# Darkbblue/generic-diffusion-feature

Hardware: AMD Instinct MI355X
Metric: images/sec feature-extract, SDXL 1024^2 single-timestep (higher is better)
Workload: dtype f16; 1 GPU; SDXL UNet 1024x1024 (latent 128x128), batch 16/GPU, t=100, hooks=config_xl_practical (4 ids, 15.73 MB/img), full forward; global_batch=16, parallelism=dp1 (batch sharded, weights broadcast once), residual_stream=fp32 master + fp16 shadow, launched_by=single process, max_inflight_forwards=0

## Files before the change

generic-diffusion-feature_amd/csrc/gemm.hip:

```cpp
#include "gemm_mainloop_ring.h"
#include "gemm_mainloop_8phase.h"
#include "gemm_epilogue.h"
#include <cstdio>
#include <cstdlib>
#include <cstring>
#include <deque>
#include <mutex>
#include <string>

namespace gdf {

template <int MODE, int BM, int BN, int STAGES, bool GEGLU, bool DIT, bool BF = false, bool QKN = false, bool SPLIT = false, bool MX = false,
          bool GNS = false>
__device__ __forceinline__ void gemm_body(const GemmParams& p) {
  using T = GemmTile<MODE, BM, BN, STAGES, GEGLU, DIT, BF, QKN, SPLIT, MX, GNS>;
  extern __shared__ __attribute__((aligned(16))) char smem[];
  T t(p, smem);
  const int tiles_n = (p.N + BN - 1) / BN;
  const int nblk = ((p.M + BM - 1) / BM) * tiles_n;
  constexpr bool PERSIST = (STAGES == 8);
  int vb = blockIdx.x;
#if defined(GDF_STAGGER)
  if (p.stagger > 0 && (int)blockIdx.x < p.stagger_wgs) {
    const unsigned long long t0 = __builtin_amdgcn_s_memrealtime();
    const unsigned long long d = (unsigned long long)(p.stagger & 0xffffff) * (unsigned)((blockIdx.x >> 3) % (unsigned)(p.stagger >> 24));
    while (__builtin_amdgcn_s_memrealtime() - t0 < d) __builtin_amdgcn_s_sleep(16);
  }
#endif
  do {
  GDF_TR(0); GDF_TR_ID();
  t.locate(vb, tiles_n, nblk);
  f32x4 acc[T::FM][T::FN];
#pragma unroll
  for (int i = 0; i < T::FM; ++i)
#pragma unroll
    for (int j = 0; j < T::FN; ++j) acc[i][j] = f32x4{0.f, 0.f, 0.f, 0.f};
  if constexpr (STAGES == 8) gemm_mainloop_8phase_256(t, acc);
  else if constexpr (STAGES == 9) gemm_mainloop_8phase_320(t, acc);
  else gemm_mainloop_ring(t, acc);
#if defined(GDF_ABLATE_EPI) && GDF_ABLATE_EPI == 2
  wait_vmcnt<0>();
#endif
  __syncthreads();
  GDF_TR(3);
#if defined(GDF_ABLATE_EPI) && GDF_ABLATE_EPI == 1
#pragma unroll
  for (int i = 0; i < T::FM; ++i)
#pragma unroll
    for (int j = 0; j < T::FN; ++j) asm volatile("" ::"v"(acc[i][j]));
#else
  gemm_epilogue(t, acc);
#endif
  GDF_TR(4);
  if constexpr (!PERSIST) break;
  vb += gridDim.x;
  if (vb >= nblk) break;
  asm volatile("s_waitcnt lgkmcnt(0)" ::: "memory");
  __builtin_amdgcn_s_barrier();
  } while (true);
}

template <int MODE, int BM, int BN, int STAGES, bool GEGLU>
__global__ __launch_bounds__(BM * 2, 2) void gemm_kernel(const GemmParams p) {
  gemm_body<MODE, BM, BN, STAGES, GEGLU, false>(p);
}
template <int MODE, int BM, int BN, int STAGES>
__global__ __launch_bounds__(BM * 2, 2) void gemm_gn_kernel(const GemmParams p) {
  gemm_body<MODE, BM, BN, STAGES, false, false, false, false, false, false, true>(p);
}
template <int MODE, int BM, int BN, int STAGES, bool GEGLU>
__global__ __launch_bounds__(BM * 2, 2) void gemm_split_kernel(const GemmParams p) {
  gemm_body<MODE, BM, BN, STAGES, GEGLU, false, false, false, true>(p);
}
template <int BM, int BN, int STAGES, bool BF, bool QKN>
__global__ __launch_bounds__(BM * 2, 2) void gemm_dit_kernel(const GemmParams p) {
  gemm_body<A_DENSE, BM, BN, STAGES, false, true, BF, QKN>(p);
}

template <int BM, int BN, int STAGES, bool BF, bool QKN>
__global__ __launch_bounds__(BM * 2, 2) void gemm_dit_split_kernel(const GemmParams p) {
  gemm_body<A_DENSE, BM, BN, STAGES, false, true, BF, QKN, true>(p);
}

template <int BM, int BN, int STAGES>
__global__ __launch_bounds__(BM * 2, 2) void gemm_mx_kernel(const GemmParams p) {
  gemm_body<A_DENSE, BM, BN, STAGES, false, true, true, false, false, true>(p);
}

static int persist_wgs() {
  static const int off = [] { const char* e = getenv("GDF_PERSIST"); return e && atoi(e) == 0; }();
  if (off) return 1 << 30;
  static std::atomic<int> cus[16];
  int dev = 0;
  if (hipGetDevice(&dev) != hipSuccess || dev < 0 || dev >= 16) return 1 << 30;
  int n = cus[dev].load(std::memory_order_relaxed);
  if (n == 0) {
    if (hipDeviceGetAttribute(&n, hipDeviceAttributeMultiprocessorCount, dev) != hipSuccess || n < 8 || (n & 7)) n = 1 << 30;
    cus[dev].store(n, std::memory_order_relaxed);
  }
  return n;
}

template <int MODE, int BM, int BN, int STAGES, bool GEGLU, bool DIT = false, bool BF = false, bool QKN = false, bool SPLIT = false, bool MX = false,
          bool GNS = false>
static hipError_t launch_t(const GemmParams& p, hipStream_t s) {
  const int tiles_m = (p.M + BM - 1) / BM, tiles_n = (p.N + BN - 1) / BN;
  const int smem = (STAGES >= 8 ? 2 : STAGES) * (BM * 128 + BN * 128);
  static std::atomic<uint64_t> attr_mask{0};
  {
    const void* fn;
    if constexpr (MX) fn = (const void*)gemm_mx_kernel<BM, BN, STAGES>;
    else if constexpr (GNS) fn = (const void*)gemm_gn_kernel<MODE, BM, BN, STAGES>;
    else if constexpr (DIT && SPLIT) fn = (const void*)gemm_dit_split_kernel<BM, BN, STAGES, BF, QKN>;
    else if constexpr (DIT) fn = (const void*)gemm_dit_kernel<BM, BN, STAGES, BF, QKN>;
    else if constexpr (SPLIT) fn = (const void*)gemm_split_kernel<MODE, BM, BN, STAGES, GEGLU>;
    else fn = (const void*)gemm_kernel<MODE, BM, BN, STAGES, GEGLU>;
    const hipError_t e = ensure_dyn_smem(attr_mask, fn, smem);
    if (e != hipSuccess) return e;
  }
  GemmParams q = p;
  q.sb_gm = q.sb_gn = 0;
  if (!p.no_superblock) {
    const int conc = (p.cus > 0 ? p.cus / 8 : 32) * ((BM == 256) ? 1 : 2);
    static const int gn_max = [] { const char* e = getenv("GDF_SB_GN_MAX"); return e ? atoi(e) : 4; }();
    for (int gn = gn_max; gn >= 2; gn >>= 1) {
      const int gm = conc / gn;
      if (tiles_n % gn == 0 && tiles_m % gm == 0 && (tiles_m / gm) * (tiles_n / gn) >= 8 && tiles_n > gn) {
        q.sb_gm = gm; q.sb_gn = gn;
        break;
      }
    }
  }
  int gx = tiles_m * tiles_n;
  const int pw = (p.cus > 0 && p.cus < persist_wgs()) ? p.cus : persist_wgs();
  {
    static const float us = [] { const char* e = getenv("GDF_STAGGER_US"); return e ? (float)atof(e) : 0.f; }();
    static const int min_rounds = [] { const char* e = getenv("GDF_STAGGER_MIN_ROUNDS"); return e ? atoi(e) : 2; }();
    q.stagger = 0; q.stagger_wgs = 0;
    static const int groups = [] { const char* e = getenv("GDF_STAGGER_GROUPS"); return e ? atoi(e) : 2; }();
    if (us > 0.f && groups > 1 && BM == 256 && pw < (1 << 30) && gx >= min_rounds * pw) { q.stagger = (int)(us * 100.f) | (groups << 24); q.stagger_wgs = pw; }
  }
  if (STAGES == 8 && gx > pw && !(p.batch > 1)) gx = pw;
  const dim3 grid(gx, (STAGES == 2 && p.splitk > 1) ? p.splitk : p.batch > 1 ? p.batch : 1);
  if constexpr (MX) hipLaunchKernelGGL((gemm_mx_kernel<BM, BN, STAGES>), grid, dim3(BM * 2), smem, s, q);
  else if constexpr (GNS) hipLaunchKernelGGL((gemm_gn_kernel<MODE, BM, BN, STAGES>), grid, dim3(BM * 2), smem, s, q);
  else if constexpr (DIT && SPLIT) hipLaunchKernelGGL((gemm_dit_split_kernel<BM, BN, STAGES, BF, QKN>), grid, dim3(BM * 2), smem, s, q);
  else if constexpr (DIT) hipLaunchKernelGGL((gemm_dit_kernel<BM, BN, STAGES, BF, QKN>), grid, dim3(BM * 2), smem, s, q);
  else if constexpr (SPLIT) hipLaunchKernelGGL((gemm_split_kernel<MODE, BM, BN, STAGES, GEGLU>), grid, dim3(BM * 2), smem, s, q);
  else hipLaunchKernelGGL((gemm_kernel<MODE, BM, BN, STAGES, GEGLU>), grid, dim3(BM * 2), smem, s, q);
  return hipGetLastError();
}

static double round_fill(long tiles, int slots) {
  if (tiles <= 0) return 0.0;
  const long rounds = (tiles + slots - 1) / slots;
  return (double)tiles / (double)(rounds * slots);
}

static int pick_variant_any(const GemmParams& p);
static bool is_split(const GemmParams& p) { return !p.dit && (p.k_w > 0 || p.o16_lo > 0); }
static bool is_dit_split(const GemmParams& p) { return p.dit && (p.k_w > 0 || p.o16_lo > 0); }
static int pick_variant(const GemmParams& p) {
  const int v = pick_variant_any(p);
  if (is_dit_split(p)) return (v == 8256 || v == 1256) ? 8256 : 128;
  if (!is_split(p) || v == 16) return v;
  if (p.geglu) return v == 825 ? 825 : 128;
  if (p.mode == A_CONV_SMALLC) return v == 160 ? 160 : 128;
  return (v == 932 || v == 160) ? v : 128;
}
static int pick_variant_any(const GemmParams& p) {
  const int S1 = p.cus > 0 ? p.cus : 256, S2 = 2 * S1;
  if (p.dit) {
    const long t256 = (long)((p.M + 255) / 256) * ((p.N + 255) / 256);
    if (p.variant == 128 || p.variant == 1256 || p.variant == 2128 || p.variant == 8256) return p.variant;
    if (t256 >= 128 && (long)((p.N + 255) / 256) * 256 <= (long)p.N + p.N / 8) return 8256;
    return (p.N % 128 == 0 && (long)((p.M + 255) / 256) * (p.N / 128) >= 256) ? 2128 : 128;
  }
  if (p.bn == 16) return 16;
  if (p.splitk > 1) {
    static const int force = [] { const char* e = getenv("GDF_SPLITK_TILE"); return e ? atoi(e) : 0; }();
    if (force == 160 && p.N % 160 == 0) return 160;
    if (force == 128 && p.N % 128 == 0) return 128;
    return (p.N % 160 == 0) ? 160 : 128;
  }
  if (p.variant) return p.variant;
  const long tiles256 = (long)((p.M + 255) / 256) * ((p.N + 127) / 128);
  const long tiles320 = (long)((p.M + 255) / 256) * ((p.N + 319) / 320);
  if (p.geglu) {
    const long tm256 = (p.M + 255) / 256, tm128 = (p.M + 127) / 128;
    double best = 0.0; int bv = 128;
    auto cand = [&](int v, double rate, long tiles, int slots) { const double sc = rate * round_fill(tiles, slots); if (sc > best) { best = sc; bv = v; } };
    if (p.N % 256 == 0) cand(825, 1.00, tm256 * (p.N / 256), S1);
    if (p.N % 320 == 0) cand(320, 0.95, tm256 * (p.N / 320), S1);
    cand(256, 0.80, tm256 * ((p.N + 127) / 128), S1);
    cand(128, 0.70, tm128 * ((p.N + 127) / 128), S2);
// ... 4 lines not shown
      const double s932 = 1.00 * round_fill(tiles320, S1), s160 = 0.85 * round_fill((long)((p.M + 127) / 128) * (p.N / 160), S2);
      const double s128 = 0.70 * round_fill((long)((p.M + 127) / 128) * ((p.N + 127) / 128), S2);
      return (s932 >= s160 && s932 >= s128) ? 932 : (s160 >= s128 ? 160 : 128);
    }
    if (p.N % 160 == 0) return 160;
    if (p.N % 256 == 0 && (long)((p.M + 255) / 256) * (p.N / 256) >= 256) return 826;
    return (p.N <= 128 && p.M >= (1 << 20)) ? 256 : 128;
  }
  if (p.res32 && p.K <= 1536 && p.N % 160 == 0 && tiles320 <= S2 &&
      !(p.N % 320 == 0 && p.N >= 640 && p.K >= 640 && tiles320 % S1 == 0)) return 160;
  if (p.N % 320 == 0) {
    const double s932 = 1.00 * round_fill(tiles320, S1), s160 = 0.87 * round_fill((long)((p.M + 127) / 128) * (p.N / 160), S2);
    const double s128 = 0.72 * round_fill((long)((p.M + 127) / 128) * ((p.N + 127) / 128), S2);
    return (s932 >= s160 && s932 >= s128) ? 932 : (s160 >= s128 ? 160 : 128);
  }
  if (p.N % 160 == 0 && p.K >= 1024) return 160;
  if ((long)p.M * p.N >= (1L << 26) && tiles256 >= S2) return 256;
  return 128;
}

bool gemm_qkn_ok(int M, int N, int K) {
  GemmParams g{}; g.M = M; g.N = N; g.K = K; g.dit = 1; g.mode = A_DENSE;
  const int v = pick_variant(g);
  return v == 8256 || v == 1256;
}

const char* gemm_kernel_name(const GemmParams& p) {
  const int v = pick_variant(p);
  int bm = 128, bn = 128, st = 2;
  if (v == 16) bn = 16; else if (v == 160) bn = 160; else if (v == 256) { bm = 256; st = 3; } else if (v == 320) { bm = 256; bn = 320; }
  else if (v == 825) { bm = 256; bn = 256; st = 8; } else if (v == 932) { bm = 256; bn = 320; st = 9; } else if (v == 826) { bm = 256; bn = 256; st = 8; }
  if (p.mode == A_CONV_SMALLC && v != 160) { bm = 128; bn = 128; st = 2; }
  char tmp[64];
  if (p.gn_partial && !p.dit) snprintf(tmp, sizeof tmp, "gemm_gn_kernel<%d, %d, %d, %d>", p.mode, bm, bn, st);
  else if (p.dit && p.mx) snprintf(tmp, sizeof tmp, "gemm_mx_kernel<256, 256, 8>");
  else if (p.dit) snprintf(tmp, sizeof tmp, "%s<%d, %d, %d, %s, %s>", is_dit_split(p) ? "gemm_dit_split_kernel" : "gemm_dit_kernel", v == 128 ? 128 : 256, (v == 1256 || v == 8256) ? 256 : 128, v == 8256 ? 8 : v == 2128 ? 3 : 2, p.bf16 ? "true" : "false", p.qkn_nq ? "true" : "false");
  else snprintf(tmp, sizeof tmp, "%s<%d, %d, %d, %d, %s>", is_split(p) ? "gemm_split_kernel" : "gemm_kernel", p.mode, bm, bn, st, p.geglu ? "true" : "false");
  static std::mutex mu;
  static std::deque<std::string> names;
  std::lock_guard<std::mutex> lk(mu);
  for (const std::string& n : names) if (n == tmp) return n.c_str();
  names.emplace_back(tmp);
  return names.back().c_str();
}

int gemm_gn_slab_rows(const GemmParams& p) {
  if ((p.mode != A_CONV3 && p.mode != A_CONV_SMALLC) || p.dit || p.geglu || p.splitk > 1 || p.batch > 1 || is_split(p) || p.bn == 16) return 0;
  if ((p.M % 64) != 0 || (p.N % 8) != 0) return 0;
  const int v = pick_variant(p);
  if (p.mode == A_CONV_SMALLC) return v != 160 ? 64 : 0;
  if (v == 932) return (p.M % 128) == 0 ? 128 : 0;
  return (v == 128 || v == 160 || v == 256 || v == 826) ? 64 : 0;
}

hipError_t launch_gemm(const GemmParams& p, hipStream_t s) {
  if (p.M <= 0 || p.N <= 0) return hipSuccess;
  if (p.mode != A_CONV_SMALLC && (p.K % BK) != 0) return hipErrorInvalidValue;
  if (p.mode == A_CONV3 && (p.Cin % BK) != 0) return hipErrorInvalidValue;
  if (p.k_w > 0 && (p.K != 2 * p.k_w || (p.k_w % BK) != 0 || p.mode == A_CONV_SMALLC || (p.dit && !p.bf16) || (p.mode == A_CONV3 && (p.k_w % (9 * BK)) != 0)))
    return hipErrorInvalidValue;
  if (p.o16_lo > 0 && ((p.dit && !p.bf16) || p.bn == 16 || (p.o16_lo % 8) != 0)) return hipErrorInvalidValue;
  if (p.out_f16 && !(p.dit && p.bf16)) return hipErrorInvalidValue;
  const int v = pick_variant(p);
  if (v != 16 && ((p.geglu ? p.N / 2 : p.N) % 8) != 0) return hipErrorInvalidValue;
  if (p.bf16 && !p.dit) return hipErrorInvalidValue;
  if (p.gn_partial) {
    if (gemm_gn_slab_rows(p) == 0 || !p.out16) return hipErrorInvalidValue;
    if (p.mode == A_CONV_SMALLC) return launch_t<A_CONV_SMALLC, 128, 128, 2, false, false, false, false, false, false, true>(p, s);
    if (v == 932) return launch_t<A_CONV3, 256, 320, 9, false, false, false, false, false, false, true>(p, s);
    if (v == 160) return launch_t<A_CONV3, 128, 160, 2, false, false, false, false, false, false, true>(p, s);
    if (v == 826) return launch_t<A_CONV3, 256, 256, 8, false, false, false, false, false, false, true>(p, s);
    if (v == 256) return launch_t<A_CONV3, 256, 128, 3, false, false, false, false, false, false, true>(p, s);
    return launch_t<A_CONV3, 128, 128, 2, false, false, false, false, false, false, true>(p, s);
  }
  if (p.dit) {
    if (p.mode != A_DENSE || p.geglu || p.batch > 1) return hipErrorInvalidValue;
    if (p.qkn_nq && ((v != 8256 && v != 1256) || (p.qkn_nq % 128) != 0)) return hipErrorInvalidValue;
    if (p.qkn_nq && (p.res32 || p.res16 || p.rowvec || p.aux16 || p.out32)) return hipErrorInvalidValue;
    if (p.mx) {
      if (!p.bf16 || p.qkn_nq || is_dit_split(p) || (p.N % 8)) return hipErrorInvalidValue;
      return launch_t<A_DENSE, 256, 256, 8, false, true, true, false, false, true>(p, s);
    }
    if (is_dit_split(p)) {
      if (v == 8256) return p.qkn_nq ? launch_t<A_DENSE, 256, 256, 8, false, true, true, true, true>(p, s) : launch_t<A_DENSE, 256, 256, 8, false, true, true, false, true>(p, s);
      return p.qkn_nq ? hipErrorInvalidValue : launch_t<A_DENSE, 128, 128, 2, false, true, true, false, true>(p, s);
    }
    if (p.bf16) {
      if (v == 8256) return p.qkn_nq ? launch_t<A_DENSE, 256, 256, 8, false, true, true, true>(p, s) : launch_t<A_DENSE, 256, 256, 8, false, true, true>(p, s);
      if (v == 1256) return p.qkn_nq ? launch_t<A_DENSE, 256, 256, 2, false, true, true, true>(p, s) : launch_t<A_DENSE, 256, 256, 2, false, true, true>(p, s);
      if (v == 2128) return launch_t<A_DENSE, 256, 128, 3, false, true, true>(p, s);
      return launch_t<A_DENSE, 128, 128, 2, false, true, true>(p, s);
    }
    if (v == 8256) return p.qkn_nq ? launch_t<A_DENSE, 256, 256, 8, false, true, false, true>(p, s) : launch_t<A_DENSE, 256, 256, 8, false, true>(p, s);
    if (v == 1256) return p.qkn_nq ? launch_t<A_DENSE, 256, 256, 2, false, true, false, true>(p, s) : launch_t<A_DENSE, 256, 256, 2, false, true>(p, s);
    if (v == 2128) return launch_t<A_DENSE, 256, 128, 3, false, true>(p, s);
// ... 154 lines not shown
```

generic-diffusion-feature_amd/csrc/gemm_epilogue.h:

```cpp
#pragma once
#include "gemm_tile.h"

namespace gdf {

template <class T>
__device__ __forceinline__ void gemm_epilogue(T& t, f32x4 (&acc)[T::FM][T::FN]) {
  GDF_TILE_GEOMETRY(T);
  GDF_TILE_STATE(t);
  _Float16* const out16 = t.out16;
  const float* const e_res32 = QKN ? nullptr : p.res32;
  const float* const e_rowvec = QKN ? nullptr : p.rowvec;
  const _Float16* const e_res16 = QKN ? nullptr : p.res16;
  _Float16* const e_aux16 = QKN ? nullptr : p.aux16;
  float* const e_out32 = QKN ? nullptr : (STAGES == 2 && p.splitk > 1) ? p.out32 + (size_t)blockIdx.y * p.o32_sstride : p.out32;
  static_assert(!GEGLU || (FN % 2 == 0), "GEGLU needs an even number of column fragments per wave");
  constexpr int FNV = GEGLU ? FN / 2 : FN;
  constexpr int WTNV = FNV * 16;
  constexpr int SLD = WTNV + 4;
  constexpr int PR = (FM * FN >= 32) ? 16 : 32;
  constexpr int PASSES = WTM / PR;
  constexpr int FPP = FM / PASSES;
  float* st = (float*)(smem) + wave * (PR * SLD);
  constexpr int OUTW = WTNV;
  constexpr int LPR = OUTW / 8;
// ... 269 lines not shown
            if (e_aux16) e_aux16[(size_t)row * p.ldaux + col + e] = (_Float16)x;
            if (e_res32) x += e_res32[(size_t)row * p.ldres + col + e];
            else if (e_res16) x += (float)e_res16[(size_t)row * p.ldres + col + e];
            if (out16) out16[(size_t)row * p.ldo16 + col + e] = (_Float16)x;
            if (e_out32) e_out32[(size_t)row * p.ldo32 + col + e] = x;
          }
        }
    }
    __builtin_amdgcn_wave_barrier();
    __builtin_amdgcn_sched_barrier(0);
  }
  if constexpr (GNS) {
    static_assert((WTM == 64 || WTM == 128) && PR * SLD >= 64 * 16, "one slab per wave tile");
#pragma unroll
    for (int e = 0; e < 8; ++e) { st[lane * 16 + e] = gsum[e]; st[lane * 16 + 8 + e] = gsq[e]; }
    __builtin_amdgcn_wave_barrier();
    if (lane < LPR && full && p.gn_partial && m0 + wm * WTM < p.M) {
      float a[16];
#pragma unroll
      for (int e = 0; e < 16; ++e) a[e] = 0.f;
#pragma unroll
      for (int r = 0; r < RPI; ++r)
#pragma unroll
        for (int e = 0; e < 16; ++e) a[e] += st[(r * LPR + lane) * 16 + e];
      const int slab = (m0 + wm * WTM) / WTM;
      f32x4* gp = (f32x4*)(p.gn_partial + ((size_t)slab * p.N + col) * 2);
#pragma unroll
      for (int q = 0; q < 4; ++q) gp[q] = f32x4{a[2 * q], a[8 + 2 * q], a[2 * q + 1], a[8 + 2 * q + 1]};
    }
    __builtin_amdgcn_wave_barrier();
  }
}

}
```

generic-diffusion-feature_amd/csrc/kernels.h:

```cpp
#pragma once
#include <hip/hip_runtime.h>
#include <stdint.h>
#include <atomic>
#include "launch.h"

typedef _Float16 half_t;

namespace gdf {

inline hipError_t ensure_dyn_smem(std::atomic<uint64_t>& mask, const void* fn, int bytes) {
  int dev = 0;
  hipError_t e = hipGetDevice(&dev);
  if (e != hipSuccess) return e;
  const uint64_t bit = 1ull << (dev & 63);
  if (mask.load(std::memory_order_acquire) & bit) return hipSuccess;
  e = hipFuncSetAttribute(fn, hipFuncAttributeMaxDynamicSharedMemorySize, bytes);
  if (e != hipSuccess) return e;
  mask.fetch_or(bit, std::memory_order_release);
  return hipSuccess;
}

#if defined(__HIPCC__)
__device__ __forceinline__ float e16_to_f32(half_t h, int bf) {
  return bf ? __uint_as_float((uint32_t)__builtin_bit_cast(unsigned short, h) << 16) : (float)h;
// ... 38 lines not shown
  int geglu;
  int bn;
  int splitk;
  long o32_sstride;
  int batch;
  long w_bstride;
  long o_bstride;
  int sb_gm, sb_gn;
  int no_superblock;
  int no_early_mma;
  int variant;
  int dit;
  int act;
  int rv_mul;
  int rv_seg_rows, rv_rps2;
  int rv_tok;
  int qkn_nq;
  const float* qkn_wq; const float* qkn_wk; float qkn_eps;
  const float* rope_cos; const float* rope_sin;
  int qkn_pos0, qkn_rps;
  int qkn_seg_rows, qkn_pos1, qkn_rps2;
  int bf16;
  float acc_scale, out16_scale;
  int k_w;
  uint32_t a_lo_bytes;
  int o16_lo;
  int cus;
  int out_f16;
  int mx;
  const float* mx_rowscale;
  const float* mx_colscale;
  float* gn_partial;
  int stagger, stagger_wgs;
};
hipError_t launch_gemm(const GemmParams& p, hipStream_t s);
int gemm_gn_slab_rows(const GemmParams& p);
int gemm_splitk_factor(const GemmParams& p);
hipError_t launch_gemm_splitk(const GemmParams& p, int splitk, float* ws, hipStream_t s);
const char* gemm_kernel_name(const GemmParams& p);
bool gemm_qkn_ok(int M, int N, int K);

struct AttnParams {
  const half_t* q; int ldq;
  const half_t* k; int ldk;
  const half_t* v; int ldv;
  half_t* o; int ldo;
  int B, heads, Sq, Sk, D;
  int kv_bstride;
  float scale;
  half_t* map;
  half_t* map2;
  const int* kv_len;
  int seg_T;
  int bf16;
  int o_lo;
  int o_pair_bf16;
  int q_lo, kv_lo;
  float o_scale;
};
hipError_t launch_attention(const AttnParams& p, hipStream_t s);

size_t gn_partial_floats(int B, int HW, int C);
hipError_t launch_gn_stats(const half_t* x16, const float* x32, int ld, int B, int HW, int C, int G, float eps,
                           const float* gamma, const float* beta, float* partial, float* ab, hipStream_t s, int x_lo = 0);
hipError_t launch_gn_apply(const half_t* x16, const float* x32, int ld, int B, int HW, int C,
                           const float* ab, int silu, half_t* y, hipStream_t s, int x_lo = 0, int ldy = 0, int y_lo = 0);
// ... 59 lines not shown
```

generic-diffusion-feature_amd/csrc/model.cpp:

```cpp
#include "builder.h"
#include <shared_mutex>

namespace gdf {

thread_local std::string g_err;
void set_error(const std::string& s) { g_err = s; }
const char* last_error() { return g_err.c_str(); }

struct ModelBuilder : WeightBuilder {
  explicit ModelBuilder(Model& mm) : WeightBuilder(mm) {}
  ResnetW resnet(const std::string& p, int ci, int co) {
    ResnetW r; r.cin = ci; r.cout = co;
    r.n1 = norm(p + ".norm1", ci);
    r.c1 = conv3(p + ".conv1", co, ci);
    r.temb_off = m.temb_total;
    m.temb_regs.push_back({p + ".time_emb_proj", co, m.temb_total});
    m.temb_total += co;
    r.n2 = norm(p + ".norm2", co);
    r.c2 = conv3(p + ".conv2", co, co);
    r.has_sc = ci != co;
    if (r.has_sc) r.sc = lin(p + ".conv_shortcut", co, ci, true, true);
    return r;
  }

  VitW vit(const std::string& p, int c, int heads, int depth) {
    const GdfArch& a = m.arch;
    VitW v; v.c = c; v.heads = heads;
    v.gn = norm(p + ".norm", c);
    v.pin = lin(p + ".proj_in", c, c, true, !a.use_linear_projection);
    for (int i = 0; i < depth; ++i) {
      const std::string b = p + ".transformer_blocks." + std::to_string(i);
      BlockW w;
      w.ln1 = norm(b + ".norm1", c);
      w.qkv = lin_alloc(3 * c, c, false);
// ... 213 lines not shown
    const size_t gn = groupnorm(x, w.gn, 1e-6f, false, SP_GNV);
    Act tok = new_act(C, x.H, x.W, true);
    {
      Epi e; e.bias = wt(w.pin.b); e.has_bias = true; out_to(e, tok, w.blocks.empty());
      gemm("proj_in", ws(gn), C * p_gnv, n, w.pin, C, C, 0, e, s_gnv * C);
    }
    untmp(gn, img_bytes(n, C, SP_GNV));
    for (size_t bi = 0; bi < w.blocks.size() && !stop; ++bi) {
      const BlockW& bw = w.blocks[bi];
      const std::string bid = id + "-block" + std::to_string(bi);
      const size_t nb = n * C * 2;
      const size_t nb_lna = img_bytes(n, C, SP_LN_ATTN), nb_ao = img_bytes(n, C, SP_ATTN_OUT), nb_ao2 = img_bytes(n, C, SP_ATTN2_OUT), nb_lnf = img_bytes(n, C, SP_LN_FF);
      size_t ln = layernorm(tok, bw.ln1, SP_LN_ATTN);
      const int s_qkv = spl(SP_QKV), lq = 3 * C * (1 + s_qkv);
      const size_t qkv = tmp(n * (size_t)lq * 2);
      { Epi e; e.out16 = ws(qkv); e.has_o16 = true; e.ldo16 = lq; e.o16_lo = s_qkv * 3 * C;
        gemm("attn1_qkv", ws(ln), C * p_lna, n, bw.qkv, 3 * C, C, 0, e, s_lna * C); }
      untmp(ln, nb_lna);
      hook_copy(want(bid + "-self-q", C, x.H, x.W), ws(qkv), lq, n, C);
      hook_copy(want(bid + "-self-k", C, x.H, x.W), ws(qkv + (size_t)C * 2), lq, n, C);
      hook_copy(want(bid + "-self-v", C, x.H, x.W), ws(qkv + (size_t)2 * C * 2), lq, n, C);
      size_t ao = tmp(nb_ao);
      const int ms = maps ? want_map(bid + "-self-map", heads, S, S) : (dry_map(bid + "-self-map"), -1);
      attention("attn1", ws(qkv), lq, ws(qkv + (size_t)C * 2), lq, ws(qkv + (size_t)2 * C * 2), lq, ws(ao), C * p_ao, heads,
                S, S, D, ms, -1, s_ao * C, s_qkv * 3 * C, s_qkv * 3 * C);
      untmp(qkv, n * (size_t)lq * 2);
      { Epi e; e.bias = wt(bw.o1.b); e.has_bias = true; residual_from(e, tok); out_to(e, tok, false);
        gemm("attn1_out", ws(ao), C * p_ao, n, bw.o1, C, C, 0, e, s_ao * C); }
      untmp(ao, nb_ao);
      if (stop) break;
      ln = layernorm(tok, bw.ln2, SP_LN_ATTN);
      const int s_xq = spl(SP_XQKV);
      const int hq = want(bid + "-cross-q", C, x.H, x.W);
      const bool q2_direct = hq >= 0 && !s_xq;
      const size_t q2 = q2_direct ? 0 : tmp(nb * (1 + s_xq));
      const Ref q2r = q2_direct ? Ref{BUF_HOOK0 + hq, 0} : ws(q2);
      { Epi e; e.out16 = q2r; e.has_o16 = true; e.ldo16 = C * (1 + s_xq); e.o16_lo = s_xq * C;
        gemm("attn2_q", ws(ln), C * p_lna, n, bw.q2, C, C, 0, e, s_lna * C); }
      untmp(ln, nb_lna);
      if (q2_direct) hook_done();
      else if (hq >= 0) hook_copy(hq, ws(q2), C * (1 + s_xq), n, C);
      const bool shared = opt.reserved[0] != 0;
      const size_t kv = dry ? 0 : kv_bufs[bw.kv_group].first + (size_t)bw.kv_index * kv_bufs[bw.kv_group].second;
      ao = tmp(nb_ao2);
      const int mc = maps ? want_map(bid + "-cross-map", heads, S, n_ctx) : (dry_map(bid + "-cross-map"), -1);
      attention("attn2", q2r, C * (1 + s_xq), ws(kv), 2 * C * (1 + s_xq), ws(kv + (size_t)C * 2), 2 * C * (1 + s_xq), ws(ao), C * p_ao2, heads, S, n_ctx, D, mc,
                shared ? 0 : n_ctx, s_ao2 * C, s_xq * C, s_xq * 2 * C);
      if (!q2_direct) untmp(q2, nb * (1 + s_xq));
      { Epi e; e.bias = wt(bw.o2.b); e.has_bias = true; residual_from(e, tok); out_to(e, tok, false);
        gemm("attn2_out", ws(ao), C * p_ao2, n, bw.o2, C, C, 0, e, s_ao2 * C); }
      untmp(ao, nb_ao2);
      if (stop) break;
      ln = layernorm(tok, bw.ln3, SP_LN_FF);
      const int hi = want(bid + "-ffn-inner", 4 * C, x.H, x.W);
      const bool direct = hi >= 0 && !s_inn;
      const size_t inner_b = img_bytes(n, 4 * C, SP_FF_INNER);
      const size_t inner = direct ? 0 : tmp(inner_b);
      const Ref innr = direct ? Ref{BUF_HOOK0 + hi, 0} : ws(inner);
      { Epi e; e.bias = wt(bw.ff1.b); e.has_bias = true; e.geglu = geglu_group(8 * C); e.out16 = innr; e.has_o16 = true; e.ldo16 = 4 * C * p_inn;
        e.o16_lo = s_inn * 4 * C;
        gemm("ff_geglu", ws(ln), C * p_lnf, n, bw.ff1, 8 * C, C, 0, e, s_lnf * C); }
      untmp(ln, nb_lnf);
      if (direct) hook_done();
      else if (hi >= 0) hook_copy(hi, innr, 4 * C * p_inn, n, 4 * C);
      {
        const bool shadow = (bi + 1 == w.blocks.size()) || (!dry && P.requested.count(bid + "-out"));
        Epi e; e.bias = wt(bw.ff2.b); e.has_bias = true; residual_from(e, tok); out_to(e, tok, shadow);
        gemm("ff_out", innr, 4 * C * p_inn, n, bw.ff2, C, 4 * C, 0, e, s_inn * 4 * C); }
      if (!direct) untmp(inner, inner_b);
      gather(bid + "-out", tok);
    }
    if (!stop) {
      Epi e; e.bias = wt(w.pout.b); e.has_bias = true; residual_from(e, x); out_to(e, y);
      gemm("proj_out", tok.h, tok.ld, n, w.pout, C, C, 0, e, tok.lo);
    }
    free_act(tok);
    gather(id + "-out", y);
  }
  void dry_map(const std::string& id) { if (dry) P.dry_ids.push_back(id); }

  size_t layernorm(const Act& x, const NormW& w, int out_cls) {
// ... 504 lines not shown
```

generic-diffusion-feature_amd/csrc/ops_api.cpp:

```cpp
#include "../../include/gdf_ops.h"
#include "model.h"

using namespace gdf;

static bool span_ok(size_t a_bytes, size_t w_bytes, const char* what) {
  if (a_bytes < (1ull << 31) && w_bytes < (1ull << 31)) return true;
  set_error(std::string(what) + ": operand larger than 2 GiB (32-bit buffer offsets); split the rows");
  return false;
}

static int fin(hipError_t e, const char* what) {
  if (e == hipSuccess) return GDF_OK;
  set_error(std::string(what) + ": " + hipGetErrorString(e));
  return GDF_ERR_HIP;
}

extern "C" {

int gdf_op_gemm(const void* A, int lda, const void* W, const float* bias, const float* res32, const void* res16,
                int ldres, void* out16, int ldo16, float* out32, int ldo32, int M, int N, int K, int flags,
                void* stream) {
  GemmParams g{};
  if (!span_ok(((size_t)M - 1) * lda * 2 + (size_t)K * 2, (size_t)N * K * 2, "gemm")) return GDF_ERR_UNSUPPORTED;
  g.A = (const half_t*)A; g.lda = lda; g.a_bytes = (uint32_t)(((size_t)M - 1) * lda * 2 + (size_t)K * 2);
// ... 113 lines not shown

int gdf_op_splitk_factor(int M, int N, int K, int conv) {
  GemmParams g{}; g.M = M; g.N = N; g.K = K; g.mode = conv ? A_CONV3 : A_DENSE; g.bn = 128;
  return gemm_splitk_factor(g);
}

int gdf_op_conv_in(const void* x_nchw, int B, int Cin, int H, int W, const void* w_oihw, const float* bias, int Cout,
                   void* out16, void* scratch, void* stream) {
  hipStream_t s = (hipStream_t)stream;
  half_t* lat8 = (half_t*)scratch;
  half_t* w = (half_t*)((char*)scratch + (size_t)B * H * W * 16);
  hipError_t e = launch_pack_latents((const half_t*)x_nchw, B, Cin, H, W, lat8, nullptr, s);
  if (e != hipSuccess) return fin(e, "pack_latents");
  e = launch_relayout_conv(w_oihw, 0, w, Cout, Cin, 9, 8, 16, s);
  if (e != hipSuccess) return fin(e, "relayout");
  GemmParams g{};
  const size_t M = (size_t)B * H * W;
  g.A = lat8; g.lda = 8; g.a_bytes = (uint32_t)(M * 16);
  g.M = (int)M; g.N = Cout; g.K = 128; g.mode = A_CONV_SMALLC; g.H = H; g.W = W; g.OH = H; g.OW = W; g.stride = 1; g.Cin = 8;
  g.Wt = w; g.w_bytes = (uint32_t)((size_t)Cout * 256);
  g.bias = bias; g.out16 = (half_t*)out16; g.ldo16 = Cout; g.bn = 128; g.rows_per_sample = 1;
  return fin(launch_gemm(g, s), "conv_in");
}

int gdf_op_attention(const void* q, int ldq, const void* k, int ldk, const void* v, int ldv, void* o, int ldo,
                     int B, int heads, int Sq, int Sk, int D, void* map, void* stream) {
  AttnParams a{};
  a.q = (const half_t*)q; a.ldq = ldq; a.k = (const half_t*)k; a.ldk = ldk; a.v = (const half_t*)v; a.ldv = ldv;
  a.o = (half_t*)o; a.ldo = ldo; a.B = B; a.heads = heads; a.Sq = Sq; a.Sk = Sk; a.D = D; a.kv_bstride = Sk;
  a.scale = 1.0f / sqrtf((float)D); a.map = (half_t*)map;
  return fin(launch_attention(a, (hipStream_t)stream), "attention");
}

size_t gdf_op_groupnorm_scratch_bytes(int B, int HW, int C) { return gn_partial_floats(B, HW, C) * 4 + (size_t)B * C * 8 + 256; }

int gdf_op_groupnorm(const void* x16, const float* x32, int ld, int B, int HW, int C, int G, float eps,
                     const float* gamma, const float* beta, int silu, void* y, void* scratch, void* stream) {
  hipStream_t s = (hipStream_t)stream;
  if (gn_fused_slab(B, HW, C, G))
    return fin(launch_gn_fused((const half_t*)x16, x32, ld, B, HW, C, G, eps, gamma, beta, silu, (half_t*)y, s), "gn_fused");
  float* partial = (float*)scratch;
  float* ab = partial + (gn_partial_floats(B, HW, C) + 63) / 64 * 64;
  hipError_t e = launch_gn_stats((const half_t*)x16, x32, ld, B, HW, C, G, eps, gamma, beta, partial, ab, s);
  if (e != hipSuccess) return fin(e, "gn_stats");
  return fin(launch_gn_apply((const half_t*)x16, x32, ld, B, HW, C, ab, silu, (half_t*)y, s), "gn_apply");
}

int gdf_op_layernorm(const void* x16, const float* x32, int ld, int R, int C, float eps, const float* gamma,
                     const float* beta, void* y, void* stream) {
  return fin(launch_layernorm((const half_t*)x16, x32, ld, R, C, eps, gamma, beta, (half_t*)y, (hipStream_t)stream), "layernorm");
}

int gdf_op_copy2d(const void* s16, const float* s32, int lds, void* dst, int ldd, int R, int C, void* stream) {
  return fin(launch_copy2d((const half_t*)s16, s32, lds, (half_t*)dst, ldd, R, C, (hipStream_t)stream), "copy2d");
}

int gdf_op_relayout_conv3(const void* w, void* dst, int O, int I, void* stream) {
  return fin(launch_relayout_conv(w, 0, (half_t*)dst, O, I, 9, I, 9, (hipStream_t)stream, 64), "relayout_conv3");
}
int gdf_op_relayout_geglu(const void* w, const float* bias, void* w_dst, float* bias_dst, int R, int K, int group, void* stream) {
  hipError_t e = launch_relayout_rows(w, 0, (half_t*)w_dst, R, K, 0, group, (hipStream_t)stream);
  if (e != hipSuccess) return fin(e, "relayout_geglu");
  if (bias) e = launch_relayout_vec(bias, 1, bias_dst, R, 0, group, (hipStream_t)stream);
  return fin(e, "relayout_geglu_bias");
}

// ... 93 lines not shown
```

include/gdf_ops.h:

```cpp
#ifndef GDF_OPS_H
#define GDF_OPS_H
#include <stddef.h>
#include <stdint.h>
#ifdef __cplusplus
extern "C" {
#endif

int gdf_op_gemm(const void* A, int lda, const void* W, const float* bias, const float* res32, const void* res16,
                int ldres, void* out16, int ldo16, float* out32, int ldo32, int M, int N, int K, int flags,
                void* stream);

int gdf_op_conv3x3(const void* x, int ld, int B, int H, int W, int Cin, const void* Wt, int Cout, const float* bias,
                   const float* rowvec, int stride, int ups, const float* res32, void* aux16, void* out16,
                   float* out32, int narrow , void* stream);

int gdf_op_gemm_split(const void* A, int lda, int a_lo, const void* W, const float* bias, const float* res32, int ldres, void* out16,
                      int ldo16, int o16_lo, float* out32, int ldo32, int M, int N, int Kw, int flags , void* stream);
int gdf_op_conv3x3_split(const void* x, int ld, int a_lo, int B, int H, int W, int Cin, const void* Wt, int Cout, const float* bias,
                         int stride, int ups, const float* res32, void* out16, int ldo16, int o16_lo, float* out32, void* stream);
int gdf_op_layernorm_split(const float* x32, int ld, int R, int C, float eps, const float* gamma, const float* beta, void* y, int ldy,
                           int y_lo, void* stream);
int gdf_op_groupnorm_split(const void* x16, int x_lo, const float* x32, int ld, int B, int HW, int C, int G, float eps, const float* gamma,
                           const float* beta, int silu, void* y, int ldy, int y_lo, void* scratch, void* stream);
int gdf_op_attention_split(const void* q, int ldq, const void* k, int ldk, const void* v, int ldv, void* o, int ldo, int o_lo, int B,
                           int heads, int Sq, int Sk, int D, void* map, void* stream);

int gdf_op_attention_pair(const void* q, int ldq, const void* k, int ldk, const void* v, int ldv, int qkv_lo, void* o, int ldo, int o_lo, int B,
                          int heads, int Sq, int Sk, int D, void* stream);

int gdf_op_conv3x3_splitk(const void* x, int ld, int B, int H, int W, int Cin, const void* Wt, int Cout, const float* bias,
                          const float* rowvec, int stride, int ups, const float* res32, void* aux16, void* out16,
                          float* out32, int splitk, float* ws, void* stream);
int gdf_op_splitk_factor(int M, int N, int K, int conv);

int gdf_op_conv_in(const void* x_nchw, int B, int Cin, int H, int W, const void* w_oihw, const float* bias, int Cout,
                   void* out16, void* scratch, void* stream);

int gdf_op_attention(const void* q, int ldq, const void* k, int ldk, const void* v, int ldv, void* o, int ldo,
                     int B, int heads, int Sq, int Sk, int D, void* map, void* stream);

size_t gdf_op_groupnorm_scratch_bytes(int B, int HW, int C);
int gdf_op_groupnorm(const void* x16, const float* x32, int ld, int B, int HW, int C, int G, float eps,
                     const float* gamma, const float* beta, int silu, void* y, void* scratch, void* stream);

int gdf_op_layernorm(const void* x16, const float* x32, int ld, int R, int C, float eps, const float* gamma,
                     const float* beta, void* y, void* stream);

int gdf_op_copy2d(const void* s16, const float* s32, int lds, void* dst, int ldd, int R, int C, void* stream);

int gdf_op_relayout_conv3(const void* w_oihw_f16, void* dst, int O, int I, void* stream);
int gdf_op_relayout_geglu(const void* w_f16, const float* bias, void* w_dst, float* bias_dst, int R, int K, int group , void* stream);

int gdf_op_small_linear(const float* x, int ldx, int M, int K, const void* W, const float* bias, int N, int silu_in,
                        int accumulate, float* out, int ldo, void* stream);

int gdf_op_softmax_rows(void* x, int ld, int R, int n, float scale, void* stream);

int gdf_op_sincos_pos_embed(float* out, int C, int gh, int gw, int base_size, float interpolation_scale, void* stream);


int gdf_op_resize_concat(const void* src, int src_f32, long sb, long sc, long sy, long sx, int B, int C, int H, int W, void* out,
                         int Ctot, int coff, int S, void* stream);
int gdf_op_avg_pool(const void* src, long sb, long sy, long sx, int B, int C, int H, int W, int r, void* out, void* stream);
int gdf_op_maps_mean(const void* const* maps, int n, int B, int heads, int Q, int K, float* out, void* stream);


int gdf_op_set_e16(int dtype);

int gdf_op_quant_rows_fp8(const void* x16, int ld, int R, int K, int src_bf16, void* q8, int ldq, float* scale, void* stream);
int gdf_op_gemm_mx(const void* A8, int lda, const float* a_scale, const void* W8, const float* w_scale, const float* bias, int act,
                   const float* res32, int ldres, void* out16, int ldo16, float* out32, int ldo32, int M, int N, int K, void* stream);

// ... 20 lines not shown
```

Before: 149.3 images/s.

## Fuse cross-attention into the Q-projection GEMM epilogue for short text contexts

Adds a GEMM variant (256x320 tile) whose epilogue takes the freshly computed Q tile, loads the shared K/V for up to 80 context tokens into LDS, and computes softmax(QK^T)V per head with MFMA. This runs in place of the separate q2 projection plus attention kernel. It removes the Q round-trip through global memory and one kernel launch per transformer block. The cost is a heavier epilogue with extra LDS traffic and barriers, and the path is limited to D=64, shared KV, n_ctx<=80, and no cross-attention map hooks.

```diff
diff --git a/generic-diffusion-feature_amd/csrc/gemm.hip b/generic-diffusion-feature_amd/csrc/gemm.hip
--- a/generic-diffusion-feature_amd/csrc/gemm.hip
+++ b/generic-diffusion-feature_amd/csrc/gemm.hip
@@ -11,7 +11,7 @@
 namespace gdf {
 
 template <int MODE, int BM, int BN, int STAGES, bool GEGLU, bool DIT, bool BF = false, bool QKN = false, bool SPLIT = false, bool MX = false,
-          bool GNS = false>
+          bool GNS = false, bool XA = false>
 __device__ __forceinline__ void gemm_body(const GemmParams& p) {
   using T = GemmTile<MODE, BM, BN, STAGES, GEGLU, DIT, BF, QKN, SPLIT, MX, GNS>;
   extern __shared__ __attribute__((aligned(16))) char smem[];
@@ -49,7 +49,8 @@
 #pragma unroll
     for (int j = 0; j < T::FN; ++j) asm volatile("" ::"v"(acc[i][j]));
 #else
-  gemm_epilogue(t, acc);
+  if constexpr (XA) gemm_xattn_epilogue(t, acc);
+  else gemm_epilogue(t, acc);
 #endif
   GDF_TR(4);
   if constexpr (!PERSIST) break;
@@ -85,6 +86,10 @@
 template <int BM, int BN, int STAGES>
 __global__ __launch_bounds__(BM * 2, 2) void gemm_mx_kernel(const GemmParams p) {
   gemm_body<A_DENSE, BM, BN, STAGES, false, true, true, false, false, true>(p);
+}
+template <int BM, int BN, int STAGES>
+__global__ __launch_bounds__(BM * 2, 2) void gemm_xattn_kernel(const GemmParams p) {
+  gemm_body<A_DENSE, BM, BN, STAGES, false, false, false, false, false, false, false, true>(p);
 }
 
 static int persist_wgs() {
@@ -102,7 +107,7 @@
 }
 
 template <int MODE, int BM, int BN, int STAGES, bool GEGLU, bool DIT = false, bool BF = false, bool QKN = false, bool SPLIT = false, bool MX = false,
-          bool GNS = false>
+          bool GNS = false, bool XA = false>
 static hipError_t launch_t(const GemmParams& p, hipStream_t s) {
   const int tiles_m = (p.M + BM - 1) / BM, tiles_n = (p.N + BN - 1) / BN;
   const int smem = (STAGES >= 8 ? 2 : STAGES) * (BM * 128 + BN * 128);
@@ -110,6 +115,7 @@
   {
     const void* fn;
     if constexpr (MX) fn = (const void*)gemm_mx_kernel<BM, BN, STAGES>;
+    else if constexpr (XA) fn = (const void*)gemm_xattn_kernel<BM, BN, STAGES>;
     else if constexpr (GNS) fn = (const void*)gemm_gn_kernel<MODE, BM, BN, STAGES>;
     else if constexpr (DIT && SPLIT) fn = (const void*)gemm_dit_split_kernel<BM, BN, STAGES, BF, QKN>;
     else if constexpr (DIT) fn = (const void*)gemm_dit_kernel<BM, BN, STAGES, BF, QKN>;
@@ -143,6 +149,7 @@
   if (STAGES == 8 && gx > pw && !(p.batch > 1)) gx = pw;
   const dim3 grid(gx, (STAGES == 2 && p.splitk > 1) ? p.splitk : p.batch > 1 ? p.batch : 1);
   if constexpr (MX) hipLaunchKernelGGL((gemm_mx_kernel<BM, BN, STAGES>), grid, dim3(BM * 2), smem, s, q);
+  else if constexpr (XA) hipLaunchKernelGGL((gemm_xattn_kernel<BM, BN, STAGES>), grid, dim3(BM * 2), smem, s, q);
   else if constexpr (GNS) hipLaunchKernelGGL((gemm_gn_kernel<MODE, BM, BN, STAGES>), grid, dim3(BM * 2), smem, s, q);
   else if constexpr (DIT && SPLIT) hipLaunchKernelGGL((gemm_dit_split_kernel<BM, BN, STAGES, BF, QKN>), grid, dim3(BM * 2), smem, s, q);
   else if constexpr (DIT) hipLaunchKernelGGL((gemm_dit_kernel<BM, BN, STAGES, BF, QKN>), grid, dim3(BM * 2), smem, s, q);
@@ -161,6 +168,7 @@
 static bool is_split(const GemmParams& p) { return !p.dit && (p.k_w > 0 || p.o16_lo > 0); }
 static bool is_dit_split(const GemmParams& p) { return p.dit && (p.k_w > 0 || p.o16_lo > 0); }
 static int pick_variant(const GemmParams& p) {
+  if (p.xa_o) return 932;
   const int v = pick_variant_any(p);
   if (is_dit_split(p)) return (v == 8256 || v == 1256) ? 8256 : 128;
   if (!is_split(p) || v == 16) return v;
@@ -231,7 +239,8 @@
   else if (v == 825) { bm = 256; bn = 256; st = 8; } else if (v == 932) { bm = 256; bn = 320; st = 9; } else if (v == 826) { bm = 256; bn = 256; st = 8; }
   if (p.mode == A_CONV_SMALLC && v != 160) { bm = 128; bn = 128; st = 2; }
   char tmp[64];
-  if (p.gn_partial && !p.dit) snprintf(tmp, sizeof tmp, "gemm_gn_kernel<%d, %d, %d, %d>", p.mode, bm, bn, st);
+  if (p.xa_o) snprintf(tmp, sizeof tmp, "gemm_xattn_kernel<256, 320, 9>");
+  else if (p.gn_partial && !p.dit) snprintf(tmp, sizeof tmp, "gemm_gn_kernel<%d, %d, %d, %d>", p.mode, bm, bn, st);
   else if (p.dit && p.mx) snprintf(tmp, sizeof tmp, "gemm_mx_kernel<256, 256, 8>");
   else if (p.dit) snprintf(tmp, sizeof tmp, "%s<%d, %d, %d, %s, %s>", is_dit_split(p) ? "gemm_dit_split_kernel" : "gemm_dit_kernel", v == 128 ? 128 : 256, (v == 1256 || v == 8256) ? 256 : 128, v == 8256 ? 8 : v == 2128 ? 3 : 2, p.bf16 ? "true" : "false", p.qkn_nq ? "true" : "false");
   else snprintf(tmp, sizeof tmp, "%s<%d, %d, %d, %d, %s>", is_split(p) ? "gemm_split_kernel" : "gemm_kernel", p.mode, bm, bn, st, p.geglu ? "true" : "false");
@@ -260,6 +269,14 @@
     return hipErrorInvalidValue;
   if (p.o16_lo > 0 && ((p.dit && !p.bf16) || p.bn == 16 || (p.o16_lo % 8) != 0)) return hipErrorInvalidValue;
   if (p.out_f16 && !(p.dit && p.bf16)) return hipErrorInvalidValue;
+  if (p.xa_o) {
+    if (p.dit || p.mode != A_DENSE || p.geglu || p.bn == 16 || p.splitk > 1 || p.batch > 1 || p.k_w > 0 || p.o16_lo > 0 || p.gn_partial || p.bias ||
+        p.rowvec || p.res32 || p.res16 || p.out32 || p.aux16 || (p.N % 320) != 0 || p.xa_sk < 1 || p.xa_sk > 80 || !p.xa_k || !p.xa_v ||
+        (p.xa_ldkv % 8) != 0 || (p.xa_ldo % 8) != 0 || (p.out16 && (p.ldo16 % 8) != 0) ||
+        (long)p.M * p.xa_ldo >= (1L << 31) || (long)p.M * p.ldo16 >= (1L << 31))
+      return hipErrorInvalidValue;
+    return launch_t<A_DENSE, 256, 320, 9, false, false, false, false, false, false, false, true>(p, s);
+  }
   const int v = pick_variant(p);
   if (v != 16 && ((p.geglu ? p.N / 2 : p.N) % 8) != 0) return hipErrorInvalidValue;
   if (p.bf16 && !p.dit) return hipErrorInvalidValue;
diff --git a/generic-diffusion-feature_amd/csrc/gemm_epilogue.h b/generic-diffusion-feature_amd/csrc/gemm_epilogue.h
--- a/generic-diffusion-feature_amd/csrc/gemm_epilogue.h
+++ b/generic-diffusion-feature_amd/csrc/gemm_epilogue.h
@@ -325,4 +325,147 @@
   }
 }
 
+
+template <class T>
+__device__ __forceinline__ void gemm_xattn_epilogue(T& t, f32x4 (&acc)[T::FM][T::FN]) {
+  GDF_TILE_GEOMETRY(T);
+  GDF_TILE_STATE(t);
+  static_assert(BM == 256 && BN == 320 && WTM == 128 && WTN == 80 && NW == 8, "the 256x320 tile: 2 x 4 waves of 128 x 80, 5 heads of 64");
+  typedef _Float16 h16x4 __attribute__((ext_vector_type(4)));
+  constexpr int XD = 64;
+  constexpr int LQ = XD + 8;
+  constexpr int NKEY = 80;
+  constexpr int NKV = 96;
+  constexpr int LVT = NKV + 8;
+  static_assert((2 * BM * LQ + NKEY * LQ + XD * LVT) * 2 <= 2 * (BM * 128 + BN * 128), "fits the main loop's LDS");
+  _Float16* const sQ = (_Float16*)smem;
+  _Float16* const sO = sQ + BM * LQ;
+  _Float16* const sK = sO + BM * LQ;
+  _Float16* const sVt = sK + NKEY * LQ;
+  const int tid = wave * 64 + lane;
+  _Float16* const out16 = t.out16;
+  const float a_sc = p.acc_scale != 0.f ? p.acc_scale : 1.0f;
+  const float o_sc = p.out16_scale != 0.f ? p.out16_scale : 1.0f;
+  typedef _Float16 h16x2 __attribute__((ext_vector_type(2)));
+  h16x2 qh[FM][FN][2];
+#pragma unroll
+  for (int i = 0; i < FM; ++i)
+#pragma unroll
+    for (int j = 0; j < FN; ++j)
+#pragma unroll
+      for (int r = 0; r < 4; r += 2)
+        qh[i][j][r >> 1] = __builtin_convertvector(f32x2{(acc[i][j][r] * a_sc + 0.f) * o_sc, (acc[i][j][r + 1] * a_sc + 0.f) * o_sc}, h16x2);
+  const int Sk = p.xa_sk;
+  const float sl2 = p.xa_scale * 1.44269504088896340736f;
+  const int qr0 = wave * 32;
+  for (int h = 0; h < BN / XD; ++h) {
+    const int hg = n0 / XD + h;
+    __syncthreads();
+#pragma unroll
+    for (int j = 0; j < FN; ++j) {
+      const int c = wn * WTN + j * 16;
+      if ((c >> 6) == h) {
+#pragma unroll
+        for (int i = 0; i < FM; ++i)
+#pragma unroll
+          for (int r = 0; r < 4; ++r) sQ[(wm * WTM + i * 16 + fk * 4 + r) * LQ + (c & 63) + frow] = qh[i][j][r >> 1][r & 1];
+      }
+    }
+    for (int c = tid; c < NKV * 8; c += NW * 64) {
+      const int key = c >> 3, ch = (c & 7) * 8;
+      f16x8 kv = {0, 0, 0, 0, 0, 0, 0, 0}, vv = kv;
+      if (key < Sk) {
+        if (key < NKEY) kv = *(const f16x8*)(p.xa_k + (size_t)key * p.xa_ldkv + hg * XD + ch);
+        vv = *(const f16x8*)(p.xa_v + (size_t)key * p.xa_ldkv + hg * XD + ch);
+      }
+      if (key < NKEY) *(f16x8*)(sK + key * LQ + ch) = kv;
+#pragma unroll
+      for (int e = 0; e < 8; ++e) sVt[(ch + e) * LVT + key] = vv[e];
+    }
+    __syncthreads();
+    if (out16) {
+#pragma unroll
+      for (int it = 0; it < BM * 8 / (NW * 64); ++it) {
+        const int c = it * NW * 64 + tid, row = c >> 3, ch = (c & 7) * 8;
+        if (m0 + row < p.M) *(f16x8*)(out16 + hg * XD + (uint32_t)((m0 + row) * p.ldo16 + ch)) = *(const f16x8*)(sQ + row * LQ + ch);
+      }
+    }
+#pragma unroll
+    for (int a = 0; a < 2; ++a) {
+      const f16x8 q0 = *(const f16x8*)(sQ + (qr0 + 16 * a + frow) * LQ + 8 * fk);
+      const f16x8 q1 = *(const f16x8*)(sQ + (qr0 + 16 * a + frow) * LQ + 32 + 8 * fk);
+      f32x4 sc[5];
+#pragma unroll
+      for (int f = 0; f < 5; ++f) {
+        const f16x8 k0 = *(const f16x8*)(sK + (16 * f + frow) * LQ + 8 * fk);
+        const f16x8 k1 = *(const f16x8*)(sK + (16 * f + frow) * LQ + 32 + 8 * fk);
+        sc[f] = mfma16<false>(k0, q0, f32x4{0.f, 0.f, 0.f, 0.f});
+        sc[f] = mfma16<false>(k1, q1, sc[f]);
+      }
+#pragma unroll
+      for (int f = 0; f < 5; ++f)
+#pragma unroll
+        for (int r = 0; r < 4; ++r)
+          if (16 * f + 4 * fk + r >= Sk) sc[f][r] = -INFINITY;
+      float mx = sc[0][0], mx2 = sc[4][0];
+#pragma unroll
+      for (int f = 0; f < 4; ++f)
+#pragma unroll
+        for (int r = 0; r < 4; ++r) mx = fmaxf(mx, sc[f][r]);
+#pragma unroll
+      for (int r = 1; r < 4; ++r) mx2 = fmaxf(mx2, sc[4][r]);
+      mx = fmaxf(mx, __shfl_xor(mx, 16)); mx = fmaxf(mx, __shfl_xor(mx, 32));
+      mx2 = fmaxf(mx2, __shfl_xor(mx2, 16)); mx2 = fmaxf(mx2, __shfl_xor(mx2, 32));
+      const float m1 = mx * sl2, mt = mx2 * sl2;
+      const float m = (mt > m1 + 8.0f) ? mt : m1;
+      float s1 = 0.f, s2 = 0.f;
+      f16x8 pb[3];
+#pragma unroll
+      for (int f = 0; f < 5; ++f)
+#pragma unroll
+        for (int r = 0; r < 4; ++r) {
+          const float e = __builtin_amdgcn_exp2f(sc[f][r] * sl2 - (f < 4 ? m1 : m));
+          if (f < 4) s1 += e; else s2 += e;
+          pb[f >> 1][(f & 1) * 4 + r] = (_Float16)e;
+        }
+#pragma unroll
+      for (int r = 0; r < 4; ++r) pb[2][4 + r] = (_Float16)0.f;
+      s1 += __shfl_xor(s1, 16); s1 += __shfl_xor(s1, 32);
+      s2 += __shfl_xor(s2, 16); s2 += __shfl_xor(s2, 32);
+      const float alpha = __builtin_amdgcn_exp2f(m1 - m);
+      f32x4 o[4];
+#pragma unroll
+      for (int e = 0; e < 4; ++e) o[e] = f32x4{0.f, 0.f, 0.f, 0.f};
+#pragma unroll
+      for (int tt = 0; tt < 3; ++tt) {
+        if (tt == 2) {
+#pragma unroll
+          for (int e = 0; e < 4; ++e) o[e] *= alpha;
+        }
+#pragma unroll
+        for (int e = 0; e < 4; ++e) {
+          const _Float16* vp = sVt + (16 * e + frow) * LVT + 32 * tt + 4 * fk;
+          const h16x4 v0 = *(const h16x4*)vp, v1 = *(const h16x4*)(vp + 16);
+          const f16x8 va = {v0[0], v0[1], v0[2], v0[3], v1[0], v1[1], v1[2], v1[3]};
+          o[e] = mfma16<false>(va, pb[tt], o[e]);
+        }
+      }
+      const float inv = 1.0f / (s1 * alpha + s2);
+#pragma unroll
+      for (int e = 0; e < 4; ++e) {
+        h16x4 hv;
+#pragma unroll
+        for (int r = 0; r < 4; ++r) hv[r] = (_Float16)(o[e][r] * inv);
+        *(h16x4*)(sO + (qr0 + 16 * a + frow) * LQ + 16 * e + 4 * fk) = hv;
+      }
+    }
+    __builtin_amdgcn_wave_barrier();
+#pragma unroll
+    for (int it = 0; it < 4; ++it) {
+      const int row = qr0 + it * 8 + (lane >> 3), ch = (lane & 7) * 8;
+      if (m0 + row < p.M) *(f16x8*)(p.xa_o + hg * XD + (uint32_t)((m0 + row) * p.xa_ldo + ch)) = *(const f16x8*)(sO + row * LQ + ch);
+    }
+  }
 }
+
+}
diff --git a/generic-diffusion-feature_amd/csrc/kernels.h b/generic-diffusion-feature_amd/csrc/kernels.h
--- a/generic-diffusion-feature_amd/csrc/kernels.h
+++ b/generic-diffusion-feature_amd/csrc/kernels.h
@@ -94,6 +94,9 @@
   const float* mx_colscale;
   float* gn_partial;
   int stagger, stagger_wgs;
+  const half_t* xa_k; const half_t* xa_v; int xa_ldkv, xa_sk;
+  half_t* xa_o; int xa_ldo;
+  float xa_scale;
 };
 hipError_t launch_gemm(const GemmParams& p, hipStream_t s);
 int gemm_gn_slab_rows(const GemmParams& p);
diff --git a/generic-diffusion-feature_amd/csrc/model.cpp b/generic-diffusion-feature_amd/csrc/model.cpp
--- a/generic-diffusion-feature_amd/csrc/model.cpp
+++ b/generic-diffusion-feature_amd/csrc/model.cpp
@@ -1,5 +1,9 @@
 #include "builder.h"
 #include <shared_mutex>
+
+#ifndef GDF_XATTN_FUSED
+#define GDF_XATTN_FUSED 1
+#endif
 
 namespace gdf {
 
@@ -279,6 +283,28 @@
       ln = layernorm(tok, bw.ln2, SP_LN_ATTN);
       const int s_xq = spl(SP_XQKV);
       const int hq = want(bid + "-cross-q", C, x.H, x.W);
+      const bool shared = opt.reserved[0] != 0;
+      const size_t kv = dry ? 0 : kv_bufs[bw.kv_group].first + (size_t)bw.kv_index * kv_bufs[bw.kv_group].second;
+      const bool fuse = GDF_XATTN_FUSED && D == 64 && C % 320 == 0 && !s_xq && !s_lna && !s_ao2 && shared && n_ctx <= 80 &&
+                        !(maps && !dry && P.requested.count(bid + "-cross-map"));
+      if (fuse) {
+        ao = tmp(nb_ao2);
+        const Ref A = ws(ln), W = wt(bw.q2.w), K = ws(kv), V = ws(kv + (size_t)C * 2), O = ws(ao), Qh = hq >= 0 ? Ref{BUF_HOOK0 + hq, 0} : Ref{};
+        const int M = (int)n, cus = opt.reserved[2], Sk = n_ctx;
+        op("attn2_qx", 2.0 * (double)n * C * C + 4.0 * (double)n * Sk * C, [=](const Bind& b, hipStream_t s) {
+          GemmParams g{};
+          g.A = (const half_t*)b.p(A); g.lda = C; g.a_bytes = (uint32_t)(((size_t)M - 1) * C * 2 + (size_t)C * 2);
+          g.M = M; g.N = C; g.K = C; g.mode = A_DENSE; g.cus = cus; g.bn = 128;
+          g.Wt = (const half_t*)b.p(W); g.w_bytes = (uint32_t)((size_t)C * C * 2);
+          if (hq >= 0) { g.out16 = (half_t*)b.p(Qh); g.ldo16 = C; }
+          g.xa_k = (const half_t*)b.p(K); g.xa_v = (const half_t*)b.p(V); g.xa_ldkv = 2 * C; g.xa_sk = Sk;
+          g.xa_o = (half_t*)b.p(O); g.xa_ldo = C; g.xa_scale = 1.0f / sqrtf((float)D);
+          return launch_gemm(g, s);
+        }, "gemm_xattn_kernel<256, 320, 9>");
+        untmp(ln, nb_lna);
+        if (hq >= 0) hook_done();
+        if (maps) (void)want_map(bid + "-cross-map", heads, S, n_ctx); else dry_map(bid + "-cross-map");
+      } else {
       const bool q2_direct = hq >= 0 && !s_xq;
       const size_t q2 = q2_direct ? 0 : tmp(nb * (1 + s_xq));
       const Ref q2r = q2_direct ? Ref{BUF_HOOK0 + hq, 0} : ws(q2);
@@ -287,13 +313,12 @@
       untmp(ln, nb_lna);
       if (q2_direct) hook_done();
       else if (hq >= 0) hook_copy(hq, ws(q2), C * (1 + s_xq), n, C);
-      const bool shared = opt.reserved[0] != 0;
-      const size_t kv = dry ? 0 : kv_bufs[bw.kv_group].first + (size_t)bw.kv_index * kv_bufs[bw.kv_group].second;
       ao = tmp(nb_ao2);
       const int mc = maps ? want_map(bid + "-cross-map", heads, S, n_ctx) : (dry_map(bid + "-cross-map"), -1);
       attention("attn2", q2r, C * (1 + s_xq), ws(kv), 2 * C * (1 + s_xq), ws(kv + (size_t)C * 2), 2 * C * (1 + s_xq), ws(ao), C * p_ao2, heads, S, n_ctx, D, mc,
                 shared ? 0 : n_ctx, s_ao2 * C, s_xq * C, s_xq * 2 * C);
       if (!q2_direct) untmp(q2, nb * (1 + s_xq));
+      }
       { Epi e; e.bias = wt(bw.o2.b); e.has_bias = true; residual_from(e, tok); out_to(e, tok, false);
         gemm("attn2_out", ws(ao), C * p_ao2, n, bw.o2, C, C, 0, e, s_ao2 * C); }
       untmp(ao, nb_ao2);
diff --git a/generic-diffusion-feature_amd/csrc/ops_api.cpp b/generic-diffusion-feature_amd/csrc/ops_api.cpp
--- a/generic-diffusion-feature_amd/csrc/ops_api.cpp
+++ b/generic-diffusion-feature_amd/csrc/ops_api.cpp
@@ -169,6 +169,18 @@
   return fin(launch_attention(a, (hipStream_t)stream), "attention");
 }
 
+int gdf_op_gemm_xattn(const void* A, int lda, const void* W, void* q_out, int ldq, const void* k, const void* v, int ldkv, int Sk,
+                      void* o, int ldo, int M, int N, int K, void* stream) {
+  GemmParams g{};
+  if (!span_ok(((size_t)M - 1) * lda * 2 + (size_t)K * 2, (size_t)N * K * 2, "gemm_xattn")) return GDF_ERR_UNSUPPORTED;
+  g.A = (const half_t*)A; g.lda = lda; g.a_bytes = (uint32_t)(((size_t)M - 1) * lda * 2 + (size_t)K * 2);
+  g.M = M; g.N = N; g.K = K; g.mode = A_DENSE; g.bn = 128; g.rows_per_sample = 1;
+  g.Wt = (const half_t*)W; g.w_bytes = (uint32_t)((size_t)N * K * 2);
+  g.out16 = (half_t*)q_out; g.ldo16 = ldq;
+  g.xa_k = (const half_t*)k; g.xa_v = (const half_t*)v; g.xa_ldkv = ldkv; g.xa_sk = Sk; g.xa_o = (half_t*)o; g.xa_ldo = ldo; g.xa_scale = 0.125f;
+  return fin(launch_gemm(g, (hipStream_t)stream), "gemm_xattn");
+}
+
 size_t gdf_op_groupnorm_scratch_bytes(int B, int HW, int C) { return gn_partial_floats(B, HW, C) * 4 + (size_t)B * C * 8 + 256; }
 
 int gdf_op_groupnorm(const void* x16, const float* x32, int ld, int B, int HW, int C, int G, float eps,
diff --git a/include/gdf_ops.h b/include/gdf_ops.h
--- a/include/gdf_ops.h
+++ b/include/gdf_ops.h
@@ -38,6 +38,9 @@
 
 int gdf_op_attention(const void* q, int ldq, const void* k, int ldk, const void* v, int ldv, void* o, int ldo,
                      int B, int heads, int Sq, int Sk, int D, void* map, void* stream);
+
+int gdf_op_gemm_xattn(const void* A, int lda, const void* W, void* q_out, int ldq, const void* k, const void* v, int ldkv, int Sk,
+                      void* o, int ldo, int M, int N, int K, void* stream);
 
 size_t gdf_op_groupnorm_scratch_bytes(int B, int HW, int C);
 int gdf_op_groupnorm(const void* x16, const float* x32, int ld, int B, int HW, int C, int G, float eps,
```

Result: no change. 150.3 images/s (median of 6 runs) (+0.7%).
